# ecrireme/ESR-NeRF

Measured on AMD Instinct MI355X. Metric: training rays/sec at 4096 rays x 128 samples (fine stage), higher is better.
Workload: dtype f32; 1 GPU; C2: giftbox_w fine stage on the slab scene, 4096 rays x 128 samples per GPU, grid 256x256x64, s_val=20, forward + trainer loss + backward + the TV lines on every third step (no optimizer step); rays_per_gpu=4096, samples_per_ray=128, surviving_samples=524288, parallelism=dp1

## Files before the change

esr_nerf_amd/csrc/mlp_split.hip:

```cpp
#include "mlp_common.h"

#include <type_traits>

typedef _Float16 f16x8 __attribute__((ext_vector_type(8)));

#ifndef ESR_SPLIT_STAMP
#define ESR_SPLIT_STAMP(i)
#endif

namespace {

constexpr int SPW = 4;
constexpr float SPLIT_RANGE = 60000.f;
constexpr int WRING = 3;

__device__ __forceinline__ f32x16 mfma_h(f16x8 a, f16x8 b, f32x16 c)
{
    return __builtin_amdgcn_mfma_f32_32x32x16_f16(a, b, c, 0, 0, 0);
}

template <int I, int N, typename F>
__device__ __forceinline__ void sfor(F &&f)
{
    if constexpr (I < N) {
// ... 91 lines not shown
    int b0, nb;
};
constexpr int MAX_SPLIT_SEG = 3;
struct SplitBatch {
    const float *X;
    float *H[3];
    unsigned *M[3];
    unsigned *range;
    int nseg;
    SplitSeg seg[MAX_SPLIT_SEG];
};

__device__ __forceinline__ void step_barrier()
{
    __builtin_amdgcn_sched_barrier(0);
    asm volatile("" ::: "memory");
    __builtin_amdgcn_s_waitcnt(0xc07f);
    __builtin_amdgcn_s_barrier();
    asm volatile("" ::: "memory");
    __builtin_amdgcn_sched_barrier(0);
}

constexpr int split_occ(int kind) { return kind == ESR_MLP_RADIANCE ? 1 : 2; }

constexpr int SAVE_RT = -1, SAVE_NONE = 0, SAVE_MASKS = 2;

template <int KIND>
__global__ void __launch_bounds__(64 * SPW, split_occ(KIND)) mlp_fwd_split_kernel(SplitBatch AB)
{
    constexpr int SM = SAVE_RT;
#include "mlp_split_fwd_body.h"
}
template <int KIND, int SM>
__global__ void __launch_bounds__(64 * SPW, split_occ(KIND)) split_fwd_lean_kernel(SplitBatch AB)
{
#include "mlp_split_fwd_body.h"
}

struct DSplitSeg {
    const _Float16 *planes;
    int t0, t1;
    int b0, nb;
};
struct DSplitBatch {
    const float *dz;
    const unsigned *M[3];
    float *dZ[3];
    float *dX;
    float *amax;
    int nseg;
    DSplitSeg seg[2];
};

constexpr int DG_RT = 0, DG_NODZ = 1, DG_TONE_IN = 2;

struct ToneInArgs {
    const float *Xt, *g_lin, *z_off, *z_emo, *rec_w;
    const int32_t *rec_ray;
    float *dz;
    int tiles_on;
};
constexpr int TIN_ROWS = 33, TIN_XT_ROWS = 48;
constexpr int TIN_SLOTS = 17;
constexpr int tin_slot_row(int k) { return 32 * (k >> 4) + acc_row(k & 15, 0); }
constexpr int tin_chan(int row) { return row < 3 ? row : (row < 18 ? row - 3 : row - 18) / 5; }
constexpr int tin_partner(int row) { return row < 3 || row >= TIN_ROWS ? -1 : row < 18 ? row + 15 : row - 15; }
constexpr float tin_coef(int row)
{
    return row >= TIN_ROWS ? 0.f : row < 3 ? 1.f : row < 18 ? (float)(1 << ((row - 3) % 5)) : -(float)(1 << ((row - 18) % 5));
}
constexpr bool tin_pair_used(int pair)
{
    for (int k = 0; k < TIN_SLOTS; ++k) {
        const int row0 = tin_slot_row(k), row1 = row0 + 4;
        if (tin_chan(row0) * 3 + (row1 < TIN_ROWS ? tin_chan(row1) : 0) == pair) return true;
    }
    return false;
}

template <int KIND>
__global__ void __launch_bounds__(64 * SPW, split_occ(KIND)) mlp_dgrad_split_kernel(DSplitBatch AB)
{
    constexpr int MODE = DG_RT;
    const ToneInArgs TI = {};
#include "mlp_split_dgrad_body.h"
}
template <int KIND, int MODE>
__global__ void __launch_bounds__(64 * SPW, split_occ(KIND)) split_dgrad_lean_kernel(DSplitBatch AB, ToneInArgs TI)
{
    static_assert(MODE != DG_TONE_IN || KIND == ESR_MLP_TONEMAP, "the tone mapper's input stage");
#include "mlp_split_dgrad_body.h"
}

int share_blocks_split(SplitSeg *seg, int nseg, int cap = 256)
{
    int groups[MAX_SPLIT_SEG], total = 0;
    for (int k = 0; k < nseg; ++k) { groups[k] = (seg[k].t1 - seg[k].t0 + SPW - 1) / SPW; total += groups[k]; }
    const int grid = total < cap ? total : cap;
    int given = 0;
    for (int k = 0; k < nseg; ++k) {
        int n = (int)((int64_t)grid * groups[k] / (total > 0 ? total : 1));
        if (n < 1) n = 1;
        if (n > groups[k]) n = groups[k];
        seg[k].nb = n;
        given += n;
    }
    for (int guard = 0; given != grid && guard < 1024; ++guard) {
        int pick = -1;
        double best = 0.0;
        for (int k = 0; k < nseg; ++k) {
            if (given < grid) {
                if (seg[k].nb >= groups[k]) continue;
                const double load = (double)groups[k] / seg[k].nb;
                if (pick < 0 || load > best) { pick = k; best = load; }
            } else {
                if (seg[k].nb <= 1) continue;
                const double load = (double)groups[k] / (seg[k].nb - 1);
                if (pick < 0 || load < best) { pick = k; best = load; }
            }
        }
        if (pick < 0) break;
        seg[pick].nb += given < grid ? 1 : -1;
        given += given < grid ? 1 : -1;
    }
    int b0 = 0;
    for (int k = 0; k < nseg; ++k) { seg[k].b0 = b0; b0 += seg[k].nb; }
    return b0;
}

std::atomic<unsigned *> g_range_flag[16];

template <int KIND, void (*KERNEL)(SplitBatch)>
int launch_split_as(const SplitBatch &B, int grid, hipStream_t s)
{
    static std::atomic<uint64_t> optin{0};
    if (int rc = esr_lds_optin(reinterpret_cast<const void *>(KERNEL), SplitSteps<KIND>::LDS_BYTES, optin)) return rc;
    KERNEL<<<grid, 64 * SPW, SplitSteps<KIND>::LDS_BYTES, s>>>(B);
    ESR_CHECK_LAUNCH();
    return 0;
}

template <int KIND>
int launch_split_k(SplitBatch &B, hipStream_t s)
// ... 61 lines not shown
    return 0;
}

ESR_API int esr_mlp_fwd_fine_split(const float *packed32_off, const void *planes_off, const float *packed32_emo,
                                   const void *planes_emo, const float *X, int32_t t_on, int32_t t_all, float *const *H,
                                   uint32_t *const *M, int color_row_detached, float *z_off, float *z_emo, void *stream)
{
    if (t_on < 0 || t_all < t_on || !crow_ok_split(ESR_MLP_RADIANCE, color_row_detached)) return ESR_EINVAL;
    if (t_all == 0) return 0;
    if (!packed32_off || !planes_off || !packed32_emo || !planes_emo || !X || !H || !M || !z_off || !z_emo) return ESR_EINVAL;
    SplitBatch B = {};
    B.X = X;
    for (int l = 0; l < 3; ++l) {
        if (!H[l] || !M[l]) return ESR_EINVAL;
        B.H[l] = H[l]; B.M[l] = M[l];
    }
    const _Float16 *po = static_cast<const _Float16 *>(planes_off), *pe = static_cast<const _Float16 *>(planes_emo);
    int n = 0;
    if (t_on > 0) B.seg[n++] = SplitSeg{packed32_off, po, 0, t_on, 0, color_row_detached, z_off, 0, 0};
    if (t_all > t_on) B.seg[n++] = SplitSeg{packed32_off, po, t_on, t_all, 1, 0, z_off, 0, 0};
    if (t_on > 0) B.seg[n++] = SplitSeg{packed32_emo, pe, 0, t_on, 1, 0, z_emo, 0, 0};
    B.nseg = n;
    return launch_split(ESR_MLP_RADIANCE, B, esr_stream(stream));
}

namespace {
template <int KIND, auto KERNEL, typename... EXTRA>
int launch_dsplit_as(const DSplitBatch &B, int grid, hipStream_t s, EXTRA... extra)
{
    static std::atomic<uint64_t> optin{0};
    if (int rc = esr_lds_optin(reinterpret_cast<const void *>(KERNEL), SplitSteps<KIND, true>::WBYTES, optin)) return rc;
    KERNEL<<<grid, 64 * SPW, SplitSteps<KIND, true>::WBYTES, s>>>(B, extra...);
    ESR_CHECK_LAUNCH();
    return 0;
}

template <int KIND>
int launch_dsplit_k(DSplitBatch &B, hipStream_t s, const ToneInArgs *tone_in = nullptr)
{
    int groups[2], total = 0;
    for (int k = 0; k < B.nseg; ++k) { groups[k] = (B.seg[k].t1 - B.seg[k].t0 + SPW - 1) / SPW; total += groups[k]; }
    const int cap = 256 * split_occ(KIND);
    const int grid = total < cap ? total : cap;
    if (B.nseg == 1) { B.seg[0].b0 = 0; B.seg[0].nb = grid; }
    else {
        int n0 = (int)((int64_t)grid * groups[0] / total);
        if (n0 < 1) n0 = 1;
        if (n0 > groups[0]) n0 = groups[0];
        if (grid - n0 > groups[1]) n0 = grid - groups[1];
        if (grid - n0 < 1) n0 = grid - 1;
        B.seg[0].b0 = 0; B.seg[0].nb = n0; B.seg[1].b0 = n0; B.seg[1].nb = grid - n0;
    }
    if constexpr (KIND == ESR_MLP_TONEMAP) {
        if (tone_in) return launch_dsplit_as<KIND, split_dgrad_lean_kernel<KIND, DG_TONE_IN>>(B, grid, s, *tone_in);
        bool none = true;
        for (int l = 0; l < net_desc(KIND).n_layers - 1; ++l) none = none && !B.dZ[l];
        if (none) return launch_dsplit_as<KIND, split_dgrad_lean_kernel<KIND, DG_NODZ>>(B, grid, s, ToneInArgs{});
    }
    return launch_dsplit_as<KIND, mlp_dgrad_split_kernel<KIND>>(B, grid, s);
}
int launch_dsplit(int kind, DSplitBatch &B, hipStream_t s)
{
    switch (kind) {
    case ESR_MLP_RADIANCE: return launch_dsplit_k<ESR_MLP_RADIANCE>(B, s);
    case ESR_MLP_TONEMAP:  return launch_dsplit_k<ESR_MLP_TONEMAP>(B, s);
    case ESR_MLP_BRDF:     return launch_dsplit_k<ESR_MLP_BRDF>(B, s);
    case ESR_MLP_EMIT:     return launch_dsplit_k<ESR_MLP_EMIT>(B, s);
    default:               return ESR_EINVAL;
    }
}
}

ESR_API int esr_mlp_dgrad_split(int kind, const void *planes, const float *dz, int32_t t0, int32_t t1, const uint32_t *const *M,
                                float *const *dZ, float *dX, float *amax, void *stream)
{
    if (!split_kind_ok(kind) || t0 < 0 || t1 < t0) return ESR_EINVAL;
    if (t1 == t0) return 0;
    if (!planes || !dz || !M || !dZ || !dX) return ESR_EINVAL;
    DSplitBatch B = {};
    B.dz = dz; B.dX = dX; B.amax = amax;
    for (int l = 0; l < net_desc(kind).n_layers - 1; ++l) {
        if (!M[l]) return ESR_EINVAL;
        B.M[l] = M[l]; B.dZ[l] = dZ[l];
    }
    B.nseg = 1;
    B.seg[0] = DSplitSeg{static_cast<const _Float16 *>(planes), t0, t1, 0, 0};
    return launch_dsplit(kind, B, esr_stream(stream));
}

ESR_API int esr_mlp_dgrad_fine_split(const void *planes_emo, const void *planes_off, const float *dz, int32_t t_on, int32_t t_all,
                                     const uint32_t *const *M, float *const *dZ, float *dX, float *amax, void *stream)
{
    if (t_on < 0 || t_all < t_on) return ESR_EINVAL;
    if (t_all == 0) return 0;
    if (!planes_emo || !planes_off || !dz || !M || !dZ || !dX) return ESR_EINVAL;
    DSplitBatch B = {};
    B.dz = dz; B.dX = dX; B.amax = amax;
    for (int l = 0; l < 3; ++l) {
        if (!M[l]) return ESR_EINVAL;
        B.M[l] = M[l]; B.dZ[l] = dZ[l];
    }
    int n = 0;
    if (t_on > 0) B.seg[n++] = DSplitSeg{static_cast<const _Float16 *>(planes_emo), 0, t_on, 0, 0};
    if (t_all > t_on) B.seg[n++] = DSplitSeg{static_cast<const _Float16 *>(planes_off), t_on, t_all, 0, 0};
    B.nseg = n;
    return launch_dsplit(ESR_MLP_RADIANCE, B, esr_stream(stream));
}

ESR_API int esr_fine_tone_dgrad_split(const void *planes, const float *dzt, const uint32_t *Mt, const float *Xt, const float *g_lin,
                                      const float *z_off, const float *z_emo, const int32_t *rec_ray, const float *rec_w,
                                      int32_t tiles_on, int32_t tiles_all, float *dz, float *amax, void *stream)
{
    if (tiles_on < 0 || tiles_all < tiles_on) return ESR_EINVAL;
    if (tiles_all == 0) return 0;
    if (!planes || !dzt || !Mt || !Xt || !g_lin || !z_off || !z_emo || !rec_ray || !rec_w || !dz) return ESR_EINVAL;
    DSplitBatch B = {};
    B.dz = dzt; B.amax = amax; B.M[0] = Mt;
    B.nseg = 1;
    B.seg[0] = DSplitSeg{static_cast<const _Float16 *>(planes), 0, tiles_all, 0, 0};
    const ToneInArgs TI = {Xt, g_lin, z_off, z_emo, rec_w, rec_ray, dz, tiles_on};
    return launch_dsplit_k<ESR_MLP_TONEMAP>(B, esr_stream(stream), &TI);
}
```

esr_nerf_amd/csrc/mlp_split_dgrad_body.h:

```cpp
    constexpr bool STORE_DZ = MODE == DG_RT;
    constexpr int DX_STORED = (dx_rows(KIND) + 3) / 4 * 4;
    using S = SplitSteps<KIND, true>;
    constexpr NetDesc D = net_desc(KIND);
    constexpr SplitLayout L = S::L;
    constexpr int NL = S::NL, NHID = NL - 1, HT = D.hid_tiles, NS = S::NS;
    constexpr unsigned HBYTES = HT * 32 * 32 * 4, MBYTES = (HT / 2) * 256;
    static_assert((NL == 4 || NL == 2) && HT % 2 == 0 && L.ks[0] == 1 && L.tiles_out[NL - 1] == 2 && D.out_dim <= 8 && D.zrows <= 8,
                  "the four-layer nets and the tone mapper: outputs in one k-step, grid-fed input rows in two tiles");
    DSplitSeg A = AB.seg[0];
    if (AB.nseg > 1 && (int)blockIdx.x >= AB.seg[1].b0) A = AB.seg[1];
    const int blk0 = A.b0, nblk = A.nb;
    extern __shared__ __attribute__((aligned(16))) unsigned char wl[];
    const int tid = threadIdx.x, lane = tid & 63, h = lane >> 5, s_ = lane & 31;
    const int wv = __builtin_amdgcn_readfirstlane(tid >> 6);
    const int ntiles = A.t1 - A.t0, ngroups = (ntiles + SPW - 1) / SPW;
    const rsrc_t WP = make_rsrc(A.planes, (unsigned)((S::BASE_CHUNK + L.total_chunks) * 1024));
    u32x4 pre[S::PRE];
    auto stage_load = [&](auto ST) __attribute__((always_inline)) {
        constexpr int st = decltype(ST)::value, pieces = S::chunks(st) * 64, base = S::chunk0(st) * 1024;
#pragma unroll
        for (int k = 0; k < S::PRE; ++k)
            if (k * 64 * SPW < pieces) pre[k] = __builtin_amdgcn_raw_buffer_load_b128(WP, (tid + 64 * SPW * k) * 16, base, 0);
    };
    auto stage_store = [&](auto ST, unsigned char *dst) __attribute__((always_inline)) {
        constexpr int st = decltype(ST)::value, pieces = S::chunks(st) * 64;
#pragma unroll
        for (int k = 0; k < S::PRE; ++k)
            if (k * 64 * SPW < pieces && tid + 64 * SPW * k < pieces)
                *reinterpret_cast<u32x4 *>(dst + (size_t)(tid + 64 * SPW * k) * 16) = pre[k];
    };
    auto stage_piece = [&](auto ST, auto KC, unsigned char *dst) __attribute__((always_inline)) {
        constexpr int st = decltype(ST)::value, k = decltype(KC)::value, pieces = S::chunks(st) * 64;
        if constexpr (k * 64 * SPW < pieces)
            if (tid + 64 * SPW * k < pieces) *reinterpret_cast<u32x4 *>(dst + (size_t)(tid + 64 * SPW * k) * 16) = pre[k];
    };
    if constexpr (S::RES) {
        for (int i = tid; i < L.total_chunks * 64; i += 64 * SPW)
            *reinterpret_cast<u32x4 *>(wl + (size_t)i * 16) = __builtin_amdgcn_raw_buffer_load_b128(WP, i * 16, S::BASE_CHUNK * 1024, 0);
    } else {
        stage_load(std::integral_constant<int, 0>{});
        stage_store(std::integral_constant<int, 0>{}, wl);
    }
    step_barrier();

    float zn[D.zrows];
    unsigned mn[NHID][HT / 2];
    auto fetch = [&](int tg) {
        const int tt = A.t0 + tg * SPW + wv;
        const int t = tt < A.t1 ? tt : A.t1 - 1;
        const rsrc_t RZ = make_rsrc(AB.dz + (size_t)t * D.zrows * 32, D.zrows * 32 * 4);
#pragma unroll
        for (int i = 0; i < D.zrows; ++i) zn[i] = bload1(RZ, s_ * 4, i * 128);
#pragma unroll
        for (int l = 0; l < NHID; ++l)
            load_relu_mask<HT>(make_rsrc(AB.M[l] + (size_t)t * (MBYTES / 4), MBYTES), mn[l], lane);
    };
    if ((int)blockIdx.x - blk0 < ngroups) fetch((int)blockIdx.x - blk0);
    const int hvoff = tile_voff(lane);

    float wmax = 0.f;
    const float *gainp = reinterpret_cast<const float *>(A.planes + (size_t)(S::BASE_CHUNK + L.total_chunks) * 512);
    const int gbits = __builtin_amdgcn_readfirstlane(__float_as_int(*gainp));
    const int kbase = __builtin_amdgcn_readfirstlane(141 + 127 - ((gbits >> 23) & 0xff) - ((gbits & 0x7fffff) ? 1 : 0));
    for (int tg = (int)blockIdx.x - blk0, trip = 0; tg < ngroups; tg += nblk, ++trip) {
        const int par = (NS & 1) ? (trip & 1) : 0;
        const int tt = A.t0 + tg * SPW + wv;
        const bool live = tt < A.t1;
        const int t = live ? tt : A.t1 - 1;
        int hv = hvoff;
        asm volatile("" : "+v"(hv));
        float zmax = 0.f;
#pragma unroll
        for (int i = 0; i < D.out_dim; ++i) zmax = fmaxf(zmax, fabsf(zn[i]));
#pragma unroll
        for (int o = 16; o > 0; o >>= 1) zmax = fmaxf(zmax, __shfl_xor(zmax, o));
        if (live) wmax = fmaxf(wmax, zmax);
        const int ez = (__float_as_int(zmax) >> 23) & 0xff;
        const int ks = ez == 0 ? 0 : kbase - ez;
        const int kc = ks < -100 ? -100 : (ks > 100 ? 100 : ks);
        const float sc = __int_as_float((127 + kc) << 23), isc = __int_as_float((127 - kc) << 23);
        f16x8 xi1[1], xi2[1];
        {
            float v[8];
#pragma unroll
            for (int i = 0; i < 8; ++i) v[i] = (h == 0 && i < D.out_dim) ? zn[i < D.out_dim ? i : 0] * sc : 0.f;
            split8(v, xi1[0], xi2[0]);
        }
        unsigned msk[NHID][HT / 2];
#pragma unroll
        for (int l = 0; l < NHID; ++l)
#pragma unroll
            for (int w = 0; w < HT / 2; ++w) msk[l][w] = mn[l][w];
        [[maybe_unused]] int tin_ray = -1;
        [[maybe_unused]] float tin_w = 0.f, tin_x[TIN_SLOTS], tin_z[3], tin_p[9];
        if constexpr (MODE == DG_TONE_IN) {
            tin_ray = __builtin_amdgcn_raw_buffer_load_b32(make_rsrc(TI.rec_ray + (size_t)t * 32, 128), s_ * 4, 0, 0);
            tin_w = bload1(make_rsrc(TI.rec_w + (size_t)t * 32, 128), s_ * 4, 0);
            const rsrc_t RXT = make_rsrc(TI.Xt + (size_t)t * TIN_XT_ROWS * 32, TIN_XT_ROWS * 128);
#pragma unroll
            for (int k = 0; k < TIN_SLOTS; ++k) {
                const int row0 = tin_slot_row(k), row1 = row0 + 4;
                const int p0 = tin_partner(row0) < 0 ? 0 : tin_partner(row0), p1 = tin_partner(row1) < 0 ? 0 : tin_partner(row1);
                tin_x[k] = bload1(RXT, ((h ? p1 : p0) * 32 + s_) * 4, 0);
            }
            const rsrc_t RZ3 = make_rsrc((t < TI.tiles_on ? TI.z_emo : TI.z_off) + (size_t)t * 4 * 32, 3 * 128);
#pragma unroll
            for (int c = 0; c < 3; ++c) tin_z[c] = bload1(RZ3, s_ * 4, c * 128);
#pragma unroll
            for (int c = 0; c < 9; ++c) tin_p[c] = 0.f;
        }
        fetch(tg + nblk < ngroups ? tg + nblk : tg);
        f16x8 pa1[2 * HT], pa2[2 * HT], pb1[2 * HT], pb2[2 * HT];
        f32x16 am[2];
        float ev[16];
        const float wisc = SPLIT_W_INV * isc;
        const f32x16 zero16 = {0.f, 0.f, 0.f, 0.f, 0.f, 0.f, 0.f, 0.f, 0.f, 0.f, 0.f, 0.f, 0.f, 0.f, 0.f, 0.f};

        auto micro = [&](auto QC, auto IT, auto MS, f32x16 &accm, auto &o1, auto &o2) __attribute__((always_inline)) {
            constexpr int q = decltype(QC)::value, it = decltype(IT)::value, ms = decltype(MS)::value, p = ms / 3, ph = ms % 3;
            constexpr int r0 = 2 * p, jj = r0 >> 3, i0 = r0 & 7;
            if constexpr (q == NL - 1 && MODE == DG_TONE_IN) {
                if constexpr (ph == 0) {
#pragma unroll
                    for (int rr = r0; rr < r0 + 2; ++rr) {
                        const int k = 16 * it + rr, row0 = 32 * it + acc_row(rr, 0), row1 = row0 + 4;
                        if (k < TIN_SLOTS) {
                            float x = tin_x[k];
                            if (tin_partner(row0) < 0) x = h ? x : 1.f;
                            const float cf = h ? tin_coef(row1) : tin_coef(row0);
                            float &acc = tin_p[tin_chan(row0) * 3 + (row1 < TIN_ROWS ? tin_chan(row1) : 0)];
                            acc = fmaf(accm[rr], x * cf, acc);
                        }
                    }
                }
            } else if constexpr (q == NL - 1) {
                if constexpr (ph == 0 && (MODE == DG_RT || 32 * it + acc_row(r0, 0) < DX_STORED)) {
                    const float v0 = accm[r0] * wisc, v1 = accm[r0 + 1] * wisc;
                    const rsrc_t RX = make_rsrc(AB.dX + (size_t)t * 64 * 32, live ? dx_rows(KIND) / 4 * 4 * 128 + (dx_rows(KIND) % 4 ? 512 : 0) : 0);
                    asm volatile("" : "+v"(hv));
                    bstore1(RX, v0, hv + tile_soff(0, r0), it * 4096);
                    bstore1(RX, v1, hv + tile_soff(0, r0 + 1), it * 4096);
                }
            } else {
                constexpr int d = NHID - 1 - q;
                if constexpr (ph == 0) {
                    int k0, k1;
                    asm("v_bfe_i32 %0, %1, %2, 1" : "=v"(k0) : "v"(msk[d][it >> 1]), "n"((it & 1) * 16 + r0));
                    asm("v_bfe_i32 %0, %1, %2, 1" : "=v"(k1) : "v"(msk[d][it >> 1]), "n"((it & 1) * 16 + r0 + 1));
                    const int a0 = __float_as_int(accm[r0]) & k0, a1 = __float_as_int(accm[r0 + 1]) & k1;
                    if constexpr (STORE_DZ) {
                        const rsrc_t RD = make_rsrc(AB.dZ[d] + (size_t)t * (HBYTES / 4), (live && AB.dZ[d]) ? HBYTES : 0u);
                        asm volatile("" : "+v"(hv));
                        bstore1_nt(RD, __int_as_float(a0) * wisc, hv + tile_soff(0, r0), it * 4096);
                        bstore1_nt(RD, __int_as_float(a1) * wisc, hv + tile_soff(0, r0 + 1), it * 4096);
                    }
                    ev[r0] = __int_as_float(a0) * SPLIT_W_INV; ev[r0 + 1] = __int_as_float(a1) * SPLIT_W_INV;
                } else if constexpr (ph == 1) {
                    put_pair<i0>(o1[2 * it + jj], ev[r0], ev[r0 + 1]);
                } else {
                    put_residual_pair<i0>(o2[2 * it + jj], o1[2 * it + jj], ev[r0], ev[r0 + 1]);
                }
            }
        };
        auto pending = [&](auto QC, auto IT, auto U, auto NAVAILC, f32x16 &accm, auto &o1, auto &o2) __attribute__((always_inline)) {
            constexpr int u = decltype(U)::value, navail = decltype(NAVAILC)::value;
            static_assert(navail >= 3 && navail % 3 == 0, "whole register pairs per pass");
            if constexpr (u < navail)
                sfor<0, (24 + navail - 1) / navail>([&](auto KC) {
                    constexpr int msi = u + decltype(KC)::value * navail;
                    if constexpr (msi < 24) micro(QC, IT, std::integral_constant<int, msi>{}, accm, o1, o2);
                });
        };
        auto run_layer = [&](auto QC, auto &in1, auto &in2, auto &o1, auto &o2) __attribute__((always_inline)) {
            constexpr int q = decltype(QC)::value, KS = L.ks[q], NT = L.tiles_out[q], NP = L.pairs[q];
// ... 8 lines not shown
                sfor<0, (WRING - 1 < NTOT ? WRING - 1 : NTOT)>([&](auto NC) {
                    constexpr int n0 = decltype(NC)::value, t0_ = n0 / KS, j0_ = n0 % KS;
                    wb[n0][0] = mine[((t0_ * 2 + 0) * KS + j0_) * 64];
                    wb[n0][1] = mine[((t0_ * 2 + 1) * KS + j0_) * 64];
                });
                sfor<0, NTOT>([&](auto NC) {
                    constexpr int n = decltype(NC)::value, tt_ = n / KS, j = n % KS, it = 2 * p + tt_;
                    if constexpr (n + WRING - 1 < NTOT) {
                        constexpr int t2 = (n + WRING - 1) / KS, j2 = (n + WRING - 1) % KS;
                        wb[(n + WRING - 1) % WRING][0] = mine[((t2 * 2 + 0) * KS + j2) * 64];
                        wb[(n + WRING - 1) % WRING][1] = mine[((t2 * 2 + 1) * KS + j2) * 64];
                    }
                    f32x16 &m = am[it & 1];
                    const f16x8 w1 = __builtin_bit_cast(f16x8, wb[n % WRING][0]), w2 = __builtin_bit_cast(f16x8, wb[n % WRING][1]);
                    constexpr bool HAVE = it > 0 || q > 0;
                    constexpr int pq = it > 0 ? q : q - 1, pit = it > 0 ? it - 1 : (q > 0 ? L.tiles_out[q > 0 ? q - 1 : 0] - 1 : 0);
                    auto ride = [&](auto U) __attribute__((always_inline)) {
                        if constexpr (HAVE) {
                            if constexpr (it > 0) pending(std::integral_constant<int, pq>{}, std::integral_constant<int, pit>{}, U,
                                                          std::integral_constant<int, 3 * KS>{}, am[pit & 1], o1, o2);
                            else pending(std::integral_constant<int, pq>{}, std::integral_constant<int, pit>{}, U,
                                         std::integral_constant<int, 3 * (KS - 2)>{}, am[pit & 1], in1, in2);
                        }
                        if constexpr (tt_ == tin - 1 && 3 * KS >= S::PRE && !S::RES) {
                            constexpr int u_ = decltype(U)::value, first = 3 * KS - S::PRE;
                            if constexpr (u_ >= first) stage_piece(std::integral_constant<int, nxt_st>{}, std::integral_constant<int, u_ - first>{},
                                                                   wl + ((st + 1 + par) & 1) * S::BUF);
                        }
                        __builtin_amdgcn_sched_barrier(0);
                    };
                    m = mfma_h(w1, in2[j], j == 0 ? zero16 : m);
                    ride(std::integral_constant<int, 3 * j + 0>{});
                    m = mfma_h(w1, in1[j], m);
                    ride(std::integral_constant<int, 3 * j + 1>{});
                    m = mfma_h(w2, in1[j], m);
                    ride(std::integral_constant<int, 3 * j + 2>{});
                });
                if constexpr (q == NL - 1 && p == NP - 1) {
                    sfor<0, 24>([&](auto MC) {
                        micro(QC, std::integral_constant<int, NT - 1>{}, MC, am[(NT - 1) & 1], o1, o2);
                    });
                }
                if constexpr (3 * KS < S::PRE && !S::RES)
                    stage_store(std::integral_constant<int, nxt_st>{}, wl + ((st + 1 + par) & 1) * S::BUF);
                if constexpr (!S::RES) step_barrier();
            });
        };
        run_layer(std::integral_constant<int, 0>{}, xi1, xi2, pa1, pa2);
        if constexpr (NL == 4) {
            run_layer(std::integral_constant<int, 1>{}, pa1, pa2, pb1, pb2);
            run_layer(std::integral_constant<int, 2>{}, pb1, pb2, pa1, pa2);
        }
        [[maybe_unused]] float tin_g[3] = {0.f, 0.f, 0.f};
        if constexpr (MODE == DG_TONE_IN) {
#pragma unroll
            for (int c = 0; c < 3; ++c) tin_g[c] = tin_ray >= 0 ? TI.g_lin[3 * (size_t)tin_ray + c] : 0.f;
        }
        run_layer(std::integral_constant<int, NL - 1>{}, pa1, pa2, pb1, pb2);
        if constexpr (MODE == DG_TONE_IN) {
            float dzc[3];
#pragma unroll
            for (int c = 0; c < 3; ++c) {
                float a = 0.f, b = 0.f;
#pragma unroll
                for (int o = 0; o < 3; ++o) {
                    if (tin_pair_used(c * 3 + o)) a += tin_p[c * 3 + o];
                    if (tin_pair_used(o * 3 + c)) b += tin_p[o * 3 + c];
                }
                const float own = h ? b : a;
                const float sum = (own + __shfl_xor(own, 32)) * wisc;
                const float sg = tin_z[c] > 20.f ? 1.f : esr_sigmoid(tin_z[c]);
                dzc[c] = tin_ray >= 0 ? (tin_w * tin_g[c] + sum) * sg : 0.f;
            }
            const rsrc_t RDZ = make_rsrc(TI.dz + (size_t)t * 4 * 32, live ? 4 * 128 : 0);
            bstore1(RDZ, h ? dzc[2] : dzc[0], (2 * h * 32 + s_) * 4, 0);
            bstore1(RDZ, h ? 0.f : dzc[1], (2 * h * 32 + s_) * 4, 128);
        }
    }
    wmax *= fmaxf(1.f, *gainp * 0.0625f);
    if (AB.amax && lane == 0 && wmax > *reinterpret_cast<volatile float *>(AB.amax))
        atomicMax(reinterpret_cast<unsigned *>(AB.amax), __float_as_uint(wmax));
```

esr_nerf_amd/fine_engine.py:

```python
from __future__ import annotations

import ctypes as C
import functools
import math
import os
from dataclasses import dataclass
from typing import Dict, List, Optional

import torch

from . import _lib

KIND_RADIANCE, KIND_TONEMAP = _lib.MLP_RADIANCE, _lib.MLP_TONEMAP
HID = 192
X_ROWS, DX_ROWS, XT_ROWS = 104, 64, 48


def make_scene(xyz_min, xyz_max, mask_min, mask_max, world_size, mask_size, near, stepdist,
               voxel_size, act_shift, mask_thres, fast_thres, s_val, grad_feat) -> _lib.EsrScene:
    sc = _lib.EsrScene()
    for i in range(3):
        sc.xyz_min[i], sc.xyz_max[i] = float(xyz_min[i]), float(xyz_max[i])
        sc.mask_min[i], sc.mask_max[i] = float(mask_min[i]), float(mask_max[i])
    sc.gx, sc.gy, sc.gz = [int(v) for v in world_size]
# ... 87 lines not shown

    def rec_ray_now(self):
        return self.buf.get("rec_ray")

    def rec(self):
        return self.buf["rec_ray"], self.buf["rec_step"], self.buf["rec_w"], self.buf["rec_sdf"]

    def ray_buf(self, n):
        if n not in self.ray_bufs:
            self.ray_bufs[n] = {k: torch.empty(n * w, dtype=torch.int32, device=self.device)
                                for k, w in (("cnt3", 1), ("off3", 1), ("stats", 3))}
        return self.ray_bufs[n]


class _F32Only:
    def __init__(self, eng):
        self.eng = eng

    def __enter__(self):
        self.keep, self.eng.split_fwd = self.eng.split_fwd, False

    def __exit__(self, *exc):
        self.eng.split_fwd = self.keep
        return False


def _follows_forward(backward):
    @functools.wraps(backward)
    def run(self, ctx, *args, **kw):
        if ctx.f32_only and self.split_fwd:
            with self.f32_only():
                return backward(self, ctx, *args, **kw)
        return backward(self, ctx, *args, **kw)
    return run


class _PackGroup:
    def __init__(self, eng):
        self.eng = eng

    def __enter__(self):
        self.eng._pack_pending = []

    def __exit__(self, et, ev, tb):
        eng = self.eng
        jobs, eng._pack_pending = eng._pack_pending, None
        if et is None and jobs:
            eng._pack_flush(jobs)
        return False


class FineEngine:
    fused_tone_dgrad = True

    def __init__(self, device, mlp_dtype: str = "f32"):
        if mlp_dtype not in ("f32", "bf16"):
            raise ValueError("mlp_dtype must be 'f32' or 'bf16'")
        self.device = torch.device(device)
        self.bf16 = mlp_dtype == "bf16"
        self.packed16: Dict[str, torch.Tensor] = {}
        self._p16: Dict[int, C.c_void_p] = {}
        self.L = _lib.lib()
        self.ws = _Workspace(self.device, lazy=("dXt",))
        self.plan_dev = torch.zeros(8, dtype=torch.int32, device=self.device)
        self.plan_host = torch.zeros(8, dtype=torch.int32).pin_memory()
        self.packed = {
            k: torch.empty(self.L.esr_mlp_packed_floats(kind), dtype=torch.float32, device=self.device)
            for k, kind in (("off", KIND_RADIANCE), ("emo", KIND_RADIANCE), ("tone", KIND_TONEMAP))}
        self.wgrad_scratch = torch.empty(self.L.esr_mlp_wgrad_scratch_floats(), dtype=torch.float32,
                                         device=self.device)
        self._timing = False
        self._only = None
        self._events = []
        self.n_calls = 0
        self.overlap_wgrad = True
        self._side = None
        self._raw: Dict[str, tuple] = {}
        self._pack_cache: Dict[str, tuple] = {}
        self._pack_pending = None
        self._pack_batch_cache = None
        self.x16 = self.bf16
        self.split_fwd = (not self.bf16) and os.environ.get("ESR_SPLIT_FWD", "1") != "0"
        self.split_strict = os.environ.get("ESR_SPLIT_STRICT", "0") == "1"
        self.split_fallback_steps = 0
        self.packed_split: Dict[str, torch.Tensor] = {}
        self._psplit = {}
        self.range_flag = None
        self._range_host = None
        self._range_event = None
        if self.split_fwd:
            key = str(self.device)
            if key not in _RANGE_FLAGS:
                _RANGE_FLAGS[key] = torch.zeros(1, dtype=torch.int32, device=self.device)
            self.range_flag = _RANGE_FLAGS[key]
            self._range_host = torch.zeros(1, dtype=torch.int32).pin_memory()
            with torch.cuda.device(self.device):
                _lib.check(self.L.esr_mlp_split_range_flag(_lib.ptr(self.range_flag)), "esr_mlp_split_range_flag")
        self.tone_scratch = torch.empty(self.L.esr_tone_wgrad_scratch_floats(), dtype=torch.float32, device=self.device)
        self.neus_grad = False

    def _s(self):
        return _lib.stream_ptr(self.device)

    defer_overflow = False
    overflow_seen = False
    range_strict_seen = False
# ... 392 lines not shown
        L, ws, m = self.L, self.ws, ctx.march
        sp = C.byref(m.scene)
        to, ta = m.tiles_on, m.tiles_all
        g_last, g_srgb, g_lin = g_last.contiguous(), g_srgb.contiguous(), g_lin.contiguous()
        main = torch.cuda.current_stream(self.device)
        s = self._s()
        dweight = ws["dweight"] if ta > 0 else torch.zeros(32, dtype=torch.float32, device=self.device)
        overlap = self.overlap_wgrad and ta > 0
        split = not self.bf16 and self.split_fwd

        fold = ta > 0 and not self.neus_grad and grads.get("sdf") is not None

        def march_bwd(s_):
            self._march_bwd("march_bwd", m, dweight, g_last, grads["sdf"], ws["dsdf"] if fold else None, 0, s_, walk=not fold)

        def feat_bwd(s_):
            src = (_lib.EsrFeatBwdSrc * 1)()
            src[0].dX = ws["dX"].data_ptr()
            src[0].grad_color_on = grads["emo_color"].data_ptr()
            src[0].grad_color_off = grads["off_color"].data_ptr()
            src[0].t0, src[0].t1 = 0, ta
            self._run("feat_bwd", L.esr_fine_feat_bwd, sp, C.byref(ctx.feat_args), _lib.ptr(ws["X"]),
                      _lib.ptr(ws["gnorm"]), src, 1, _lib.ptr(ws["dsdf"]) if fold else None, _lib.ptr(grads["sdf"]),
                      None, None, 0, s_)

        def wgrads(s_):
            self._tone_wgrad(ws["Xt"], ws["dzt"], 0, ta, grads["tone_w"], grads["tone_b"], ctx.amax_t if split else None, s_,
                             "tone_wgrad")
            Hh, dZh = self._H(["H0", "H1", "H2"]), self._H(["dZ0", "dZ1", "dZ2"])
            keep = [Hh, dZh]
            todo = [(KIND_RADIANCE, ws["X"], Hh, dZh, ws["dz"], 0, to, "emo_w", "emo_b"),
                    (KIND_RADIANCE, ws["X"], Hh, dZh, ws["dz"], to, ta, "off_w", "off_b")]
            jobs = (_lib.EsrWgradJob * len(todo))()
            for j, (kind, X, Hs, dZs, dzs, r0, r1, gwk, gbk) in enumerate(todo):
                gwa, gba = _lib.ptr_array(grads[gwk]), _lib.ptr_array(grads[gbk])
                keep += [gwa, gba]
                jb = jobs[j]
                jb.kind, jb.color_row0, jb.t0, jb.t1 = kind, 0, r0, r1
                jb.X, jb.dz = X.data_ptr(), dzs.data_ptr()
                jb.H, jb.dZ = C.addressof(Hs), C.addressof(dZs)
                jb.gw, jb.gb = C.addressof(gwa), C.addressof(gba)
                if ctx.x16:
                    jb.X16 = ws["X16"].data_ptr()
                if split:
                    jb.amax = ctx.amax.data_ptr()
            self._run("mlp_wgrad(all)", L.esr_mlp_wgrad_batch, jobs, len(todo), 1 if self.bf16 else 0,
                      _lib.ptr(self.wgrad_scratch), self.wgrad_scratch.numel(), s_)

        if ta == 0:
            march_bwd(s)
            if after_grids is not None:
                after_grids()
            return
        self._run("composite_bwd", L.esr_fine_composite_bwd, _lib.ptr(g_srgb), _lib.ptr(g_lin), _lib.ptr(ws["rgb"]),
                  _lib.ptr(ws["lin"]), _lib.ptr(ws["rec_ray"]), _lib.ptr(ws["rec_w"]), ta, _lib.ptr(ws["dweight"]),
                  _lib.ptr(ws["dzt"]), s)
        if fold:
            march_bwd(s)
        dZt_arg = _lib.ptr_array([None])
        M = self._H(["M0", "M1", "M2"])
        dZ = self._H(["dZ0", "dZ1", "dZ2"])
        if self.bf16:
            self._run("mlp_dgrad(tone)", L.esr_mlp_dgrad_bf16, KIND_TONEMAP, self._p16[self.packed["tone"].data_ptr()],
                      _lib.ptr(ws["dzt"]), 0, ta, self._H(["Mt"]), dZt_arg, _lib.ptr(ws["dXt"]), s)
        elif split and self.fused_tone_dgrad:
            self._run("mlp_dgrad(tone)", L.esr_fine_tone_dgrad_split, _lib.ptr(self.packed_split["tone"]), _lib.ptr(ws["dzt"]),
                      _lib.ptr(ws["Mt"]), _lib.ptr(ws["Xt"]), _lib.ptr(g_lin), _lib.ptr(ws["z_off"]), _lib.ptr(ws["z_emo"]),
                      _lib.ptr(ws["rec_ray"]), _lib.ptr(ws["rec_w"]), to, ta, _lib.ptr(ws["dz"]), _lib.ptr(ctx.amax_t), s)
        elif split:
            self._run("mlp_dgrad(tone)", L.esr_mlp_dgrad_split, KIND_TONEMAP, _lib.ptr(self.packed_split["tone"]), _lib.ptr(ws["dzt"]),
                      0, ta, self._H(["Mt"]), dZt_arg, _lib.ptr(ws["dXt"]), _lib.ptr(ctx.amax_t), s)
        else:
            self._run("mlp_dgrad(tone)", L.esr_mlp_dgrad, KIND_TONEMAP, _lib.ptr(self.packed["tone"]), _lib.ptr(ws["dzt"]), 0, ta,
                      self._H(["Mt"]), dZt_arg, _lib.ptr(ws["dXt"]), s)
        if self.bf16 or not (split and self.fused_tone_dgrad):
            self._run("tone_in_bwd", L.esr_fine_tone_in_bwd, _lib.ptr(ws["dXt"]), _lib.ptr(ws["Xt"]), _lib.ptr(g_lin),
                      _lib.ptr(ws["lin"]), _lib.ptr(ws["z_off"]), _lib.ptr(ws["z_emo"]), _lib.ptr(ws["rec_ray"]),
                      _lib.ptr(ws["rec_w"]), to, ta, _lib.ptr(ws["dz"]), s)
        if self.bf16:
            pe, po = self.packed["emo"].data_ptr(), self.packed["off"].data_ptr()
            self._run("mlp_dgrad(rad)", L.esr_mlp_dgrad_fine_bf16, self._p16[pe], self._p16[po],
                      _lib.ptr(ws["dz"]), to, ta, M, dZ, _lib.ptr(ws["dX"]), s)
        elif split:
            self._run("mlp_dgrad(rad)", L.esr_mlp_dgrad_fine_split, _lib.ptr(self.packed_split["emo"]),
                      _lib.ptr(self.packed_split["off"]), _lib.ptr(ws["dz"]), to, ta, M, dZ, _lib.ptr(ws["dX"]),
                      _lib.ptr(ctx.amax), s)
        else:
            self._run("mlp_dgrad(rad)", L.esr_mlp_dgrad_fine, _lib.ptr(self.packed["emo"]), _lib.ptr(self.packed["off"]),
                      _lib.ptr(ws["dz"]), to, ta, M, dZ, _lib.ptr(ws["dX"]), s)
        if not overlap:
            feat_bwd(s)
            if not fold:
                march_bwd(s)
            if after_grids is not None:
                after_grids()
            wgrads(s)
            return
        e_dgrad = torch.cuda.Event()
        e_dgrad.record(main)
        side = self._side_stream(0)
        side.wait_event(e_dgrad)
        with torch.cuda.stream(side):
            wgrads(_lib.stream_ptr(self.device))
            e_w = torch.cuda.Event()
            e_w.record(side)
        feat_bwd(s)
        if not fold:
            march_bwd(s)
        if after_grids is not None:
            after_grids()
        main.wait_event(e_w)

    def _side_stream(self, i=0):
        if self._side is None:
            self._side = {}
        if i not in self._side:
            self._side[i] = torch.cuda.Stream(self.device)
        return self._side[i]

    def loss_fwd_bwd(self, last, srgb, lin, rgbs, white_bg=True, weight_linear=0.1, weight_entropy_last=0.001,
                     scale=1.0):
        n = last.shape[0]
        acc = getattr(self, "_loss_acc", None)
        self._loss_acc = None
        pair = acc if acc is not None and acc.device == srgb.device else torch.zeros(2, dtype=torch.float32, device=self.device)
        self.loss_pair = pair
        loss = pair[:1]
        g_srgb = torch.empty_like(srgb)
        g_lin = torch.empty_like(lin)
        g_last = torch.empty_like(last)
        self._run("loss", self.L.esr_fine_loss_fwd_bwd_dp,
                  _lib.ptr(srgb), _lib.ptr(lin), _lib.ptr(last), _lib.ptr(rgbs.contiguous()), n,
                  1.0 if white_bg else 0.0, weight_linear, weight_entropy_last,
                  scale, _lib.ptr(loss), _lib.ptr(g_srgb), _lib.ptr(g_lin), _lib.ptr(g_last), self._s())
        return loss, g_last, g_srgb, g_lin
```

include/esr_hip.h:

```cpp
#ifndef ESR_HIP_H
#define ESR_HIP_H

#include <stdint.h>

#ifdef __cplusplus
extern "C" {
#endif

#define ESR_EINVAL (-1)
#define ESR_ECAP   (-2)

#define ESR_TILE 32

#define ESR_ABI_VERSION 48
int esr_abi_version(void);
const char *esr_build_info(void);


int esr_sample_count(const float *rays_o, const float *rays_d, const float *xyz_min,
                     const float *xyz_max, float near_, float far_, float stepdist,
                     int64_t n_rays, float *t_min, float *t_max, int64_t *n_steps,
                     int64_t *cumsum, int64_t *total, void *stream);

int esr_sample_fill(const float *rays_o, const float *rays_d, const float *xyz_min,
                    const float *xyz_max, const float *t_min, const int64_t *cumsum,
                    float stepdist, int64_t n_rays, int64_t total, float *ray_pts,
                    uint8_t *mask_outbbox, int64_t *ray_id, int64_t *step_id, void *stream);

int esr_alpha2weight_fwd(const float *alpha, const int64_t *ray_id, int64_t n_pts,
                         int64_t n_rays, float *weight, float *T, float *alphainv_last,
                         int64_t *i_start, int64_t *i_end, void *stream);

int esr_alpha2weight_bwd(const float *alpha, const float *weight, const float *T,
                         const float *alphainv_last, const int64_t *i_start,
                         const int64_t *i_end, int64_t n_pts, int64_t n_rays,
                         const float *grad_weights, const float *grad_last, float *grad,
                         void *stream);

int esr_tv_add_grad(const float *param, float *grad, float wx, float wy, float wz,
                    int64_t sz_i, int64_t sz_j, int64_t sz_k, int64_t n, int dense_mode,
                    void *stream);

int esr_segment_sum(const float *src, const int64_t *index, int64_t n, int64_t c,
                    float *out, int64_t n_seg, void *stream);

int esr_sample_count_f64(const double *rays_o, const double *rays_d, const double *xyz_min, const double *xyz_max,
                         float near_, float far_, float stepdist, int64_t n_rays, double *t_min, double *t_max,
                         int64_t *n_steps, int64_t *cumsum, int64_t *total, void *stream);
int esr_sample_fill_f64(const double *rays_o, const double *rays_d, const double *xyz_min, const double *xyz_max,
                        const double *t_min, const int64_t *cumsum, float stepdist, int64_t n_rays, int64_t total,
                        double *ray_pts, uint8_t *mask_outbbox, int64_t *ray_id, int64_t *step_id, void *stream);
int esr_alpha2weight_fwd_f64(const double *alpha, const int64_t *ray_id, int64_t n_pts, int64_t n_rays, double *weight,
                             double *T, double *alphainv_last, int64_t *i_start, int64_t *i_end, void *stream);
int esr_alpha2weight_bwd_f64(const double *alpha, const double *weight, const double *T, const double *alphainv_last,
                             const int64_t *i_start, const int64_t *i_end, int64_t n_pts, int64_t n_rays,
                             const double *grad_weights, const double *grad_last, double *grad, void *stream);

int esr_infer_t_minmax(const float *rays_o, const float *rays_d, const float *xyz_min, const float *xyz_max,
                       float near_, float far_, int64_t n_rays, float *t_min, float *t_max, void *stream);
int esr_infer_n_samples(const float *rays_d, const float *t_min, const float *t_max, float stepdist, int64_t n_rays,
                        int64_t *n_samples, void *stream);
int esr_infer_ray_start_dir(const float *rays_o, const float *rays_d, const float *t_min, int64_t n_rays,
                            float *rays_start, float *rays_dir, void *stream);
int esr_sample_ndc_pts(const float *rays_o, const float *rays_d, const float *xyz_min, const float *xyz_max,
                       int32_t n_samples, int64_t n_rays, float *rays_pts, uint8_t *mask_outbbox, void *stream);
int esr_sample_bg_pts(const float *rays_o, const float *rays_d, const float *t_max, float bg_preserve, int32_t n_samples,
                      int64_t n_rays, float *rays_pts, void *stream);
// ... 160 lines not shown
    const float *X;
    const float *const *H;
    const float *const *dZ;
    const float *dz;
    float *const *gw;
    float *const *gb;
    const void *X16;
    const float *amax;
} esr_wgrad_job_t;
int esr_mlp_wgrad_batch(const esr_wgrad_job_t *jobs, int32_t n_jobs, int bf16_operands, float *scratch,
                        int64_t scratch_floats, void *stream);

int64_t esr_tone_wgrad_scratch_floats(void);
int esr_tone_wgrad_recompute(const float *Xt, const float *dzt, const float *W0, const float *b0, const float *W1,
                             int32_t t0, int32_t t1, float *gw0, float *gb0, float *gw1, float *gb1,
                             float *scratch, int64_t scratch_floats, void *stream);
int esr_tone_wgrad_recompute_bf16(const float *Xt, const float *dzt, const float *W0, const float *b0, const float *W1,
                                  int32_t t0, int32_t t1, float *gw0, float *gb0, float *gw1, float *gb1,
                                  float *scratch, int64_t scratch_floats, void *stream);
int esr_tone_wgrad_recompute_split(const float *Xt, const float *dzt, const float *W0, const float *b0, const float *W1,
                                   const float *amax, int32_t t0, int32_t t1, float *gw0, float *gb0, float *gw1,
                                   float *gb1, float *scratch, int64_t scratch_floats, void *stream);

int64_t esr_mlp_packed_bf16_elems(int kind);
int esr_mlp_pack_bf16(int kind, const esr_mlp_weights_t *w, void *packed16, void *stream);
int esr_mlp_fwd_bf16(int kind, const float *packed32, const void *packed16, const float *X, int32_t t0,
                     int32_t t1, float *const *H, uint32_t *const *M, int save, int color_row0,
                     float *zout, void *stream);
int esr_mlp_dgrad_bf16(int kind, const void *packed16, const float *dz, int32_t t0, int32_t t1,
                       const uint32_t *const *M, float *const *dZ, float *dX, void *stream);
int esr_mlp_wgrad_bf16(int kind, const float *X, int color_row0, const float *const *H,
                       const float *const *dZ, const float *dz, int32_t t0, int32_t t1,
                       float *const *gw, float *const *gb, float *scratch, int64_t scratch_floats,
                       void *stream);

int esr_fine_tone_in_fwd(const float *z_off, const float *z_emo, int32_t tiles_on,
                         int32_t tiles_all, float *lin, float *Xt, void *stream);

int esr_fine_composite_fwd(const float *zt, const float *lin, const int32_t *rec_ray,
                           const float *rec_w, int32_t tiles_all, float *rgb,
                           float *srgb_marched, float *lin_marched, void *stream);

int esr_fine_composite_bwd(const float *g_srgb, const float *g_lin, const float *rgb,
                           const float *lin, const int32_t *rec_ray, const float *rec_w,
                           int32_t tiles_all, float *dweight, float *dzt, void *stream);

int esr_fine_tone_in_bwd(const float *dXt, const float *Xt, const float *g_lin, const float *lin,
                         const float *z_off, const float *z_emo, const int32_t *rec_ray,
                         const float *rec_w, int32_t tiles_on, int32_t tiles_all, float *dz,
                         void *stream);
int esr_fine_tone_dgrad_split(const void *planes, const float *dzt, const uint32_t *Mt, const float *Xt, const float *g_lin,
                              const float *z_off, const float *z_emo, const int32_t *rec_ray, const float *rec_w,
                              int32_t tiles_on, int32_t tiles_all, float *dz, float *amax, void *stream);

int esr_fine_loss_fwd_bwd_dp(const float *srgb_marched, const float *lin_marched,
                             const float *alphainv_last, const float *rgbs, int32_t n_rays,
                             float white_bg, float weight_linear, float weight_entropy_last, float scale,
                             float *loss, float *g_srgb, float *g_lin, float *g_last,
                             void *stream);

int esr_pair_loss_fwd_bwd(const float *a, const float *b, int64_t rows, int32_t cols,
                          const uint8_t *row_mask, int mask_value, const int32_t *count_dev,
                          int kind, float w_value, float w_a, float w_b, float *loss, float *ga,
                          float *gb, void *stream);


int esr_expgrad_fwd(const esr_scene_t *scene, const float *rays_o, const float *rays_d,
                    const int32_t *rec_ray, const int32_t *rec_step, const float *pts,
                    const float *noise, float eps, const float *sdf, int32_t n, int zero_pad,
                    float *out, void *stream);
int esr_expgrad_bwd(const esr_scene_t *scene, const float *rays_o, const float *rays_d,
                    const int32_t *rec_ray, const int32_t *rec_step, const float *pts,
                    const float *noise, float eps, const float *g, int32_t n, int zero_pad,
                    float *grad_sdf, void *stream);

int esr_lts_ref_order(const int32_t *rec_ray, const int32_t *cnt3, const int32_t *off3, const int64_t *cnt3_cumsum,
                      int32_t n_slots, int64_t *perm, int64_t *ray64, void *stream);
int esr_lts_perturb(const float *pts_all, const int64_t *perm, const float *noise_normal, const float *noise_emit,
                    float emit_eps, int32_t m3, float *noise_n, float *pts_e, void *stream);
int esr_lts_gather_rows(const float *src, int32_t tile_rows, int32_t row_stride, int32_t col0, int32_t n_ch,
                        const int64_t *perm, int32_t n, float *out, void *stream);
typedef struct esr_lts_gather {
    const int64_t *jp, *ray64;
    const float *pts_all, *eg, *rec_sdf, *viewdirs, *brdf_a, *emit_a;
    const uint8_t *umask_rays;
    int32_t n_pts;
    float *pts2, *vd2, *sdf2, *normal, *base, *rough, *metal, *emis;
    uint8_t *umask;
    int32_t *pt1;
} esr_lts_gather_t;
int esr_lts_gather_points(const esr_lts_gather_t *g, void *stream);

int esr_lts_dirs(const float *raw, const float *normal, int32_t n_pts, int32_t rays_plus_one,
                 float *dirs, void *stream);

typedef struct esr_lts_args {
    int32_t n_pts, n_rays, n_sg, pdra_mode;
    const float *base, *rough, *metal;
    const float *normal, *view;
    const float *dirs;
    const float *off_m, *emo_m, *last2;
    const float *mus, *lambdas, *lobes;
    const float *emission;
    const uint8_t *umask;
} esr_lts_args_t;

// ... 489 lines not shown
```

Before: 2.053 million rays/s.

## Fuse composite backward into the split tone-mapper dgrad kernel

Adds a DG_TONE_COMP mode to the split tone-mapper dgrad kernel. It computes the composite backward (dzt from g_srgb and rgb, and dweight from rgb, g_srgb, g_lin and lin) inside the same kernel, so the separate composite_bwd launch and the dzt round-trip through memory are no longer needed. The per-ray gradient gathers for the next tile are issued early, and the march backward is moved after the radiance dgrad. This adds register pressure and more scattered gathers to an MFMA-heavy kernel.

```diff
diff --git a/esr_nerf_amd/csrc/mlp_split.hip b/esr_nerf_amd/csrc/mlp_split.hip
--- a/esr_nerf_amd/csrc/mlp_split.hip
+++ b/esr_nerf_amd/csrc/mlp_split.hip
@@ -167,13 +167,15 @@
     DSplitSeg seg[2];
 };
 
-constexpr int DG_RT = 0, DG_NODZ = 1, DG_TONE_IN = 2;
+constexpr int DG_RT = 0, DG_NODZ = 1, DG_TONE_IN = 2, DG_TONE_COMP = 3;
 
 struct ToneInArgs {
     const float *Xt, *g_lin, *z_off, *z_emo, *rec_w;
     const int32_t *rec_ray;
     float *dz;
     int tiles_on;
+    const float *g_srgb, *rgb, *lin;
+    float *dzt, *dweight;
 };
 constexpr int TIN_ROWS = 33, TIN_XT_ROWS = 48;
 constexpr int TIN_SLOTS = 17;
@@ -204,6 +206,13 @@
 __global__ void __launch_bounds__(64 * SPW, split_occ(KIND)) split_dgrad_lean_kernel(DSplitBatch AB, ToneInArgs TI)
 {
     static_assert(MODE != DG_TONE_IN || KIND == ESR_MLP_TONEMAP, "the tone mapper's input stage");
+#include "mlp_split_dgrad_body.h"
+}
+template <int KIND>
+__global__ void __launch_bounds__(64 * SPW, split_occ(KIND)) tone_bwd_split_kernel(DSplitBatch AB, ToneInArgs TI)
+{
+    static_assert(KIND == ESR_MLP_TONEMAP, "the tone mapper's");
+    constexpr int MODE = DG_TONE_COMP;
 #include "mlp_split_dgrad_body.h"
 }
 
@@ -371,6 +380,7 @@
         B.seg[0].b0 = 0; B.seg[0].nb = n0; B.seg[1].b0 = n0; B.seg[1].nb = grid - n0;
     }
     if constexpr (KIND == ESR_MLP_TONEMAP) {
+        if (tone_in && tone_in->dzt) return launch_dsplit_as<KIND, tone_bwd_split_kernel<KIND>>(B, grid, s, *tone_in);
         if (tone_in) return launch_dsplit_as<KIND, split_dgrad_lean_kernel<KIND, DG_TONE_IN>>(B, grid, s, *tone_in);
         bool none = true;
         for (int l = 0; l < net_desc(KIND).n_layers - 1; ++l) none = none && !B.dZ[l];
@@ -437,6 +447,23 @@
     B.dz = dzt; B.amax = amax; B.M[0] = Mt;
     B.nseg = 1;
     B.seg[0] = DSplitSeg{static_cast<const _Float16 *>(planes), 0, tiles_all, 0, 0};
-    const ToneInArgs TI = {Xt, g_lin, z_off, z_emo, rec_w, rec_ray, dz, tiles_on};
+    const ToneInArgs TI = {Xt, g_lin, z_off, z_emo, rec_w, rec_ray, dz, tiles_on, nullptr, nullptr, nullptr, nullptr, nullptr};
     return launch_dsplit_k<ESR_MLP_TONEMAP>(B, esr_stream(stream), &TI);
 }
+
+ESR_API int esr_fine_tone_bwd_split(const void *planes, const float *g_srgb, const float *g_lin, const float *rgb, const float *lin,
+                                    const uint32_t *Mt, const float *Xt, const float *z_off, const float *z_emo,
+                                    const int32_t *rec_ray, const float *rec_w, int32_t tiles_on, int32_t tiles_all, float *dweight,
+                                    float *dzt, float *dz, float *amax, void *stream)
+{
+    if (tiles_on < 0 || tiles_all < tiles_on) return ESR_EINVAL;
+    if (tiles_all == 0) return 0;
+    if (!planes || !g_srgb || !g_lin || !rgb || !lin || !Mt || !Xt || !z_off || !z_emo || !rec_ray || !rec_w || !dweight || !dzt || !dz)
+        return ESR_EINVAL;
+    DSplitBatch B = {};
+    B.amax = amax; B.M[0] = Mt;
+    B.nseg = 1;
+    B.seg[0] = DSplitSeg{static_cast<const _Float16 *>(planes), 0, tiles_all, 0, 0};
+    const ToneInArgs TI = {Xt, g_lin, z_off, z_emo, rec_w, rec_ray, dz, tiles_on, g_srgb, rgb, lin, dzt, dweight};
+    return launch_dsplit_k<ESR_MLP_TONEMAP>(B, esr_stream(stream), &TI);
+}
diff --git a/esr_nerf_amd/csrc/mlp_split_dgrad_body.h b/esr_nerf_amd/csrc/mlp_split_dgrad_body.h
--- a/esr_nerf_amd/csrc/mlp_split_dgrad_body.h
+++ b/esr_nerf_amd/csrc/mlp_split_dgrad_body.h
@@ -1,4 +1,5 @@
     constexpr bool STORE_DZ = MODE == DG_RT;
+    constexpr bool TONE_IN = MODE == DG_TONE_IN || MODE == DG_TONE_COMP, COMP = MODE == DG_TONE_COMP;
     constexpr int DX_STORED = (dx_rows(KIND) + 3) / 4 * 4;
     using S = SplitSteps<KIND, true>;
     constexpr NetDesc D = net_desc(KIND);
@@ -45,17 +46,38 @@
 
     float zn[D.zrows];
     unsigned mn[NHID][HT / 2];
+    [[maybe_unused]] int cn_ray = -1;
+    [[maybe_unused]] float cn_w = 0.f, cn_col[3], gn_s[3], gn_l[3];
     auto fetch = [&](int tg) {
         const int tt = A.t0 + tg * SPW + wv;
         const int t = tt < A.t1 ? tt : A.t1 - 1;
-        const rsrc_t RZ = make_rsrc(AB.dz + (size_t)t * D.zrows * 32, D.zrows * 32 * 4);
-#pragma unroll
-        for (int i = 0; i < D.zrows; ++i) zn[i] = bload1(RZ, s_ * 4, i * 128);
+        if constexpr (COMP) {
+            cn_ray = __builtin_amdgcn_raw_buffer_load_b32(make_rsrc(TI.rec_ray + (size_t)t * 32, 128), s_ * 4, 0, 0);
+            cn_w = bload1(make_rsrc(TI.rec_w + (size_t)t * 32, 128), s_ * 4, 0);
+        } else {
+            const rsrc_t RZ = make_rsrc(AB.dz + (size_t)t * D.zrows * 32, D.zrows * 32 * 4);
+#pragma unroll
+            for (int i = 0; i < D.zrows; ++i) zn[i] = bload1(RZ, s_ * 4, i * 128);
+        }
 #pragma unroll
         for (int l = 0; l < NHID; ++l)
             load_relu_mask<HT>(make_rsrc(AB.M[l] + (size_t)t * (MBYTES / 4), MBYTES), mn[l], lane);
     };
-    if ((int)blockIdx.x - blk0 < ngroups) fetch((int)blockIdx.x - blk0);
+    [[maybe_unused]] auto gather = [&](int tg) {
+        const int tt = A.t0 + tg * SPW + wv;
+        const int t = tt < A.t1 ? tt : A.t1 - 1;
+        const rsrc_t RC = make_rsrc(TI.rgb + (size_t)t * 4 * 32, 3 * 128);
+#pragma unroll
+        for (int c = 0; c < 3; ++c) {
+            cn_col[c] = bload1(RC, s_ * 4, c * 128);
+            gn_s[c] = cn_ray >= 0 ? TI.g_srgb[3 * (size_t)cn_ray + c] : 0.f;
+            gn_l[c] = cn_ray >= 0 ? TI.g_lin[3 * (size_t)cn_ray + c] : 0.f;
+        }
+    };
+    if ((int)blockIdx.x - blk0 < ngroups) {
+        fetch((int)blockIdx.x - blk0);
+        if constexpr (COMP) gather((int)blockIdx.x - blk0);
+    }
     const int hvoff = tile_voff(lane);
 
     float wmax = 0.f;
@@ -69,6 +91,19 @@
         const int t = live ? tt : A.t1 - 1;
         int hv = hvoff;
         asm volatile("" : "+v"(hv));
+        [[maybe_unused]] float cur_lin[3] = {0.f, 0.f, 0.f};
+        if constexpr (COMP) {
+            const rsrc_t RL = make_rsrc(TI.lin + (size_t)t * 4 * 32, 3 * 128);
+#pragma unroll
+            for (int c = 0; c < 3; ++c) {
+                cur_lin[c] = bload1(RL, s_ * 4, c * 128);
+                zn[c] = cn_ray >= 0 ? cn_w * gn_s[c] * cn_col[c] * (1.f - cn_col[c]) : 0.f;
+            }
+            zn[3] = 0.f;
+            const rsrc_t RDT = make_rsrc(TI.dzt + (size_t)t * 4 * 32, live ? 4 * 128 : 0);
+            bstore1(RDT, h ? zn[2] : zn[0], (2 * h * 32 + s_) * 4, 0);
+            bstore1(RDT, h ? 0.f : zn[1], (2 * h * 32 + s_) * 4, 128);
+        }
         float zmax = 0.f;
 #pragma unroll
         for (int i = 0; i < D.out_dim; ++i) zmax = fmaxf(zmax, fabsf(zn[i]));
@@ -93,9 +128,12 @@
             for (int w = 0; w < HT / 2; ++w) msk[l][w] = mn[l][w];
         [[maybe_unused]] int tin_ray = -1;
         [[maybe_unused]] float tin_w = 0.f, tin_x[TIN_SLOTS], tin_z[3], tin_p[9];
-        if constexpr (MODE == DG_TONE_IN) {
-            tin_ray = __builtin_amdgcn_raw_buffer_load_b32(make_rsrc(TI.rec_ray + (size_t)t * 32, 128), s_ * 4, 0, 0);
-            tin_w = bload1(make_rsrc(TI.rec_w + (size_t)t * 32, 128), s_ * 4, 0);
+        if constexpr (TONE_IN) {
+            if constexpr (COMP) { tin_ray = cn_ray; tin_w = cn_w; }
+            else {
+                tin_ray = __builtin_amdgcn_raw_buffer_load_b32(make_rsrc(TI.rec_ray + (size_t)t * 32, 128), s_ * 4, 0, 0);
+                tin_w = bload1(make_rsrc(TI.rec_w + (size_t)t * 32, 128), s_ * 4, 0);
+            }
             const rsrc_t RXT = make_rsrc(TI.Xt + (size_t)t * TIN_XT_ROWS * 32, TIN_XT_ROWS * 128);
 #pragma unroll
             for (int k = 0; k < TIN_SLOTS; ++k) {
@@ -119,7 +157,7 @@
         auto micro = [&](auto QC, auto IT, auto MS, f32x16 &accm, auto &o1, auto &o2) __attribute__((always_inline)) {
             constexpr int q = decltype(QC)::value, it = decltype(IT)::value, ms = decltype(MS)::value, p = ms / 3, ph = ms % 3;
             constexpr int r0 = 2 * p, jj = r0 >> 3, i0 = r0 & 7;
-            if constexpr (q == NL - 1 && MODE == DG_TONE_IN) {
+            if constexpr (q == NL - 1 && TONE_IN) {
                 if constexpr (ph == 0) {
 #pragma unroll
                     for (int rr = r0; rr < r0 + 2; ++rr) {
@@ -234,12 +272,21 @@
             run_layer(std::integral_constant<int, 2>{}, pb1, pb2, pa1, pa2);
         }
         [[maybe_unused]] float tin_g[3] = {0.f, 0.f, 0.f};
-        if constexpr (MODE == DG_TONE_IN) {
+        if constexpr (COMP) {
+#pragma unroll
+            for (int c = 0; c < 3; ++c) tin_g[c] = gn_l[c];
+            float dw = 0.f;
+#pragma unroll
+            for (int c = 0; c < 3; ++c)
+                if (tin_ray >= 0) dw += __builtin_fmaf(cn_col[c], gn_s[c], gn_l[c] * cur_lin[c]);
+            bstore1(make_rsrc(TI.dweight + (size_t)t * 32, live ? 128 : 0), dw, h ? 128 : s_ * 4, 0);
+            gather(tg + nblk < ngroups ? tg + nblk : tg);
+        } else if constexpr (MODE == DG_TONE_IN) {
 #pragma unroll
             for (int c = 0; c < 3; ++c) tin_g[c] = tin_ray >= 0 ? TI.g_lin[3 * (size_t)tin_ray + c] : 0.f;
         }
         run_layer(std::integral_constant<int, NL - 1>{}, pa1, pa2, pb1, pb2);
-        if constexpr (MODE == DG_TONE_IN) {
+        if constexpr (TONE_IN) {
             float dzc[3];
 #pragma unroll
             for (int c = 0; c < 3; ++c) {
@@ -260,5 +307,8 @@
         }
     }
     wmax *= fmaxf(1.f, *gainp * 0.0625f);
-    if (AB.amax && lane == 0 && wmax > *reinterpret_cast<volatile float *>(AB.amax))
+    if constexpr (COMP) {
+        if (AB.amax && __builtin_amdgcn_mbcnt_hi(~0u, __builtin_amdgcn_mbcnt_lo(~0u, 0u)) == 0 && wmax > *reinterpret_cast<volatile float *>(AB.amax))
+            atomicMax(reinterpret_cast<unsigned *>(AB.amax), __float_as_uint(wmax));
+    } else if (AB.amax && lane == 0 && wmax > *reinterpret_cast<volatile float *>(AB.amax))
         atomicMax(reinterpret_cast<unsigned *>(AB.amax), __float_as_uint(wmax));
diff --git a/esr_nerf_amd/fine_engine.py b/esr_nerf_amd/fine_engine.py
--- a/esr_nerf_amd/fine_engine.py
+++ b/esr_nerf_amd/fine_engine.py
@@ -163,6 +163,8 @@
 
 class FineEngine:
     fused_tone_dgrad = True
+    fused_composite_bwd = True
+    march_bwd_late = True
 
     def __init__(self, device, mlp_dtype: str = "f32"):
         if mlp_dtype not in ("f32", "bf16"):
@@ -661,17 +663,26 @@
             if after_grids is not None:
                 after_grids()
             return
-        self._run("composite_bwd", L.esr_fine_composite_bwd, _lib.ptr(g_srgb), _lib.ptr(g_lin), _lib.ptr(ws["rgb"]),
-                  _lib.ptr(ws["lin"]), _lib.ptr(ws["rec_ray"]), _lib.ptr(ws["rec_w"]), ta, _lib.ptr(ws["dweight"]),
-                  _lib.ptr(ws["dzt"]), s)
-        if fold:
-            march_bwd(s)
+        tone_bwd = split and self.fused_tone_dgrad and self.fused_composite_bwd
+        if not tone_bwd:
+            self._run("composite_bwd", L.esr_fine_composite_bwd, _lib.ptr(g_srgb), _lib.ptr(g_lin), _lib.ptr(ws["rgb"]),
+                      _lib.ptr(ws["lin"]), _lib.ptr(ws["rec_ray"]), _lib.ptr(ws["rec_w"]), ta, _lib.ptr(ws["dweight"]),
+                      _lib.ptr(ws["dzt"]), s)
+            if fold:
+                march_bwd(s)
         dZt_arg = _lib.ptr_array([None])
         M = self._H(["M0", "M1", "M2"])
         dZ = self._H(["dZ0", "dZ1", "dZ2"])
         if self.bf16:
             self._run("mlp_dgrad(tone)", L.esr_mlp_dgrad_bf16, KIND_TONEMAP, self._p16[self.packed["tone"].data_ptr()],
                       _lib.ptr(ws["dzt"]), 0, ta, self._H(["Mt"]), dZt_arg, _lib.ptr(ws["dXt"]), s)
+        elif tone_bwd:
+            self._run("mlp_dgrad(tone)", L.esr_fine_tone_bwd_split, _lib.ptr(self.packed_split["tone"]), _lib.ptr(g_srgb), _lib.ptr(g_lin),
+                      _lib.ptr(ws["rgb"]), _lib.ptr(ws["lin"]), _lib.ptr(ws["Mt"]), _lib.ptr(ws["Xt"]), _lib.ptr(ws["z_off"]),
+                      _lib.ptr(ws["z_emo"]), _lib.ptr(ws["rec_ray"]), _lib.ptr(ws["rec_w"]), to, ta, _lib.ptr(ws["dweight"]),
+                      _lib.ptr(ws["dzt"]), _lib.ptr(ws["dz"]), _lib.ptr(ctx.amax_t), s)
+            if fold and not self.march_bwd_late:
+                march_bwd(s)
         elif split and self.fused_tone_dgrad:
             self._run("mlp_dgrad(tone)", L.esr_fine_tone_dgrad_split, _lib.ptr(self.packed_split["tone"]), _lib.ptr(ws["dzt"]),
                       _lib.ptr(ws["Mt"]), _lib.ptr(ws["Xt"]), _lib.ptr(g_lin), _lib.ptr(ws["z_off"]), _lib.ptr(ws["z_emo"]),
@@ -697,6 +708,8 @@
         else:
             self._run("mlp_dgrad(rad)", L.esr_mlp_dgrad_fine, _lib.ptr(self.packed["emo"]), _lib.ptr(self.packed["off"]),
                       _lib.ptr(ws["dz"]), to, ta, M, dZ, _lib.ptr(ws["dX"]), s)
+        if tone_bwd and fold and self.march_bwd_late:
+            march_bwd(s)
         if not overlap:
             feat_bwd(s)
             if not fold:
diff --git a/include/esr_hip.h b/include/esr_hip.h
--- a/include/esr_hip.h
+++ b/include/esr_hip.h
@@ -12,7 +12,7 @@
 
 #define ESR_TILE 32
 
-#define ESR_ABI_VERSION 48
+#define ESR_ABI_VERSION 49
 int esr_abi_version(void);
 const char *esr_build_info(void);
 
@@ -279,6 +279,10 @@
 int esr_fine_tone_dgrad_split(const void *planes, const float *dzt, const uint32_t *Mt, const float *Xt, const float *g_lin,
                               const float *z_off, const float *z_emo, const int32_t *rec_ray, const float *rec_w,
                               int32_t tiles_on, int32_t tiles_all, float *dz, float *amax, void *stream);
+int esr_fine_tone_bwd_split(const void *planes, const float *g_srgb, const float *g_lin, const float *rgb, const float *lin,
+                            const uint32_t *Mt, const float *Xt, const float *z_off, const float *z_emo,
+                            const int32_t *rec_ray, const float *rec_w, int32_t tiles_on, int32_t tiles_all, float *dweight,
+                            float *dzt, float *dz, float *amax, void *stream);
 
 int esr_fine_loss_fwd_bwd_dp(const float *srgb_marched, const float *lin_marched,
                              const float *alphainv_last, const float *rgbs, int32_t n_rays,
```

Measured after the change: 2.041 million rays/s. Within noise of the previous version (-0.6%).
